# OzAmram/CaloDiffusion

Measured on AMD Instinct MI355X. Metric: sampled showers/sec (Dataset-2, 400-step DDIM), higher is better.
Workload: dtype f32 (convs: fp32 operands as 2-term fp16 splits on the fp16 MFMA pipe, fp32 accumulate; attention/norms fp32)

## Files before the change

### calodiffusion_amd/csrc/gn_defer.h

```cpp
#pragma once
#include "kernels_gn.h"

namespace cd {

__host__ __device__ inline int gn_defer_scratch_bytes(int C) { return C * 16 + 64 * 8; }

__device__ __forceinline__ void gn_defer_to_lds(const GnDefer& g, int b, float* coef_lds, void* scratch) {
  double* sC = (double*)scratch;
  float* sMR = (float*)((char*)scratch + g.C * 16);
  const int tid = threadIdx.x, nthreads = blockDim.x;
  const int C = g.C, G = g.groups;
  float pg = 0.f, pb = 0.f, pa = 0.f;
  if (tid < C) {
    pg = g.gamma[tid];
    pb = g.beta[tid];
    pa = g.add ? g.add[(size_t)b * g.add_ld + tid] : 0.f;
  }
  for (int i = tid; i < C * 8; i += nthreads) {
    const int c = i >> 3, j = i & 7;
    const float* p = g.part + ((size_t)b * g.units * C + c) * 2;
    double a1 = 0.0, a2 = 0.0;
    for (int u = j; u < g.units; u += 32) {
      float2 v[4];
#pragma unroll
      for (int k = 0; k < 4; ++k) v[k] = u + 8 * k < g.units ? *(const float2*)(p + (size_t)(u + 8 * k) * C * 2) : float2{0.f, 0.f};
#pragma unroll
      for (int k = 0; k < 4; ++k) {
        if (u + 8 * k < g.units) {
          a1 += (double)v[k].x;
          a2 += (double)v[k].y;
        }
      }
    }
#pragma unroll
    for (int m = 1; m < 8; m <<= 1) {
      a1 += __shfl_xor(a1, m, 64);
      a2 += __shfl_xor(a2, m, 64);
    }
    if (j == 0) {
      sC[c * 2] = a1;
      sC[c * 2 + 1] = a2;
    }
  }
  __syncthreads();
  const int cpg = C / G;
  if (tid < G) {
    double a1 = 0.0, a2 = 0.0;
    for (int c = 0; c < cpg; ++c) {
      a1 += sC[(tid * cpg + c) * 2];
      a2 += sC[(tid * cpg + c) * 2 + 1];
    }
    const double cnt = (double)g.vox * cpg;
    const double mu = a1 / cnt;
    double var = a2 / cnt - mu * mu;
    var = var < 0.0 ? 0.0 : var;
    sMR[tid * 2] = (float)mu;
    sMR[tid * 2 + 1] = (float)(1.0 / sqrt(var + 1e-5));
    if (g.stat_out) {
      g.stat_out[((size_t)b * G + tid) * 2] = sMR[tid * 2];
      g.stat_out[((size_t)b * G + tid) * 2 + 1] = sMR[tid * 2 + 1];
    }
  }
  __syncthreads();
  for (int c = tid; c < C; c += nthreads) {
    const int gi = c / cpg;
    const bool pre = c == tid;
    const float sc = sMR[gi * 2 + 1] * (pre ? pg : g.gamma[c]);
    f32x4 o;
    o[0] = sc;
    o[1] = (pre ? pb : g.beta[c]) - sMR[gi * 2] * sc;
    o[2] = pre ? pa : (g.add ? g.add[(size_t)b * g.add_ld + c] : 0.f);
    o[3] = 0.f;
    *(f32x4*)(coef_lds + c * 4) = o;
    if (g.coef_out) *(f32x4*)(g.coef_out + ((size_t)b * C + c) * 4) = o;
  }
  __syncthreads();
}

}
```

### calodiffusion_amd/csrc/kernels_conv_flat16.hip

```cpp
#include "conv_internal.h"
#include "gn_defer.h"

namespace cd {

template <int VT, int CT, int KD, int KH, int KW, int SZ, int SXY, int NTERM>
__global__ void __launch_bounds__(512, (VT * CT * (NTERM == 2 ? 2 : 1) <= 2 ? 3 : 2)) conv3_flat_bf16x3_kernel(ConvFlatArgs a) {
  extern __shared__ __attribute__((aligned(16))) float lds[];
  char* ldsb = (char*)lds;
  constexpr int T = KD * KH * KW;
  constexpr int VB = NTERM == 3 ? 96 : 80;
  constexpr int WS = 64 * NTERM;
  const int tid = threadIdx.x, lane = tid & 63, wave = tid >> 6, nthreads = blockDim.x;
  const int b = blockIdx.y;
  const int ct0 = blockIdx.z * CT;
  const int HW = a.H * a.W;
  const int vox = a.D * HW;
  const int HWo = a.Ho * a.Wo;
  const int voxo = a.Do * HWo;
  const int v0 = blockIdx.x * a.R;
  const int vend = min(v0 + a.R, voxo);
  const float inv_hwo = 1.f / (float)HWo, inv_wo = 1.f / (float)a.Wo;
  auto fdiv = [](int x, float inv) { return (int)(((float)x + 0.5f) * inv); };
  const int zA = fdiv(v0, inv_hwo) * SZ - 1;
  const int zB = fdiv(vend - 1, inv_hwo) * SZ + KD - 2;
  const int nstage = (zB - zA + 1) * HW;
  const int NZ = a.P * HW;
  const int half = lane >> 5, col = lane & 31;
  if (a.defer.part) gn_defer_to_lds(a.defer, b, (float*)(ldsb + a.coef_lds_off), ldsb + a.coef_lds_off + a.defer.C * 16);
  const bool normed = a.coef || a.defer.part;
  if (tid < VB / 4) ((float*)(ldsb + (size_t)NZ * VB))[tid] = 0.f;

  int nb[VT], rowoff[VT][KH], ooff[VT];
  unsigned wmask[VT];
  bool any_valid = false;
#pragma unroll
  for (int vt = 0; vt < VT; ++vt) {
    const int v = v0 + (wave * VT + vt) * 32 + col;
    const bool valid = v < vend;
    const int vv = valid ? v : v0;
    const int oz = fdiv(vv, inv_hwo);
    const int r = vv - oz * HWo;
    const int oh = fdiv(r, inv_wo), ow = r - oh * a.Wo;
    const int ih0 = oh * SXY, iw0 = ow * SXY;
    nb[vt] = (oz * SZ - 1 - zA) * HW + ih0 * a.W + iw0;
    unsigned m = 0;
#pragma unroll
    for (int kh = 0; kh < KH; ++kh) {
      int ih = ih0 + kh - 1;
      ih = ih < 0 ? ih + a.H : (ih >= a.H ? ih - a.H : ih);
      ih = ih >= a.H ? ih - a.H : ih;
      rowoff[vt][kh] = (ih - ih0) * a.W;
    }
#pragma unroll
    for (int kw = 0; kw < KW; ++kw) {
      const int iw = iw0 + kw - 1;
      if (valid && iw >= 0 && iw < a.W) m |= 1u << kw;
    }
    wmask[vt] = m;
    ooff[vt] = valid ? v * a.cout : -1;
    any_valid |= valid;
  }
  const bool wave_active = __any(any_valid);

  f32x16 acc[VT][CT], accB[NTERM == 2 ? VT : 1][NTERM == 2 ? CT : 1];
#pragma unroll
  for (int vt = 0; vt < VT; ++vt)
#pragma unroll
    for (int ct = 0; ct < CT; ++ct)
#pragma unroll
      for (int r = 0; r < 16; ++r) {
        acc[vt][ct][r] = 0.f;
        if (NTERM == 2) accB[vt][ct][r] = 0.f;
      }

  float amax = 0.f;
  float gscale = 1.f, ginv = 1.f;
  if (NTERM == 2 && a.in_absmax) pow2_scale_for(*a.in_absmax, &gscale, &ginv);
  const int nsub = (a.c0 + a.c1) >> 4;
  const int gbase = zA * HW;
  const int nslots = nstage * 4;

  auto tap_voxel = [&](int vt, int tap) -> int {
#ifdef CD_FLAT_ABL_TAPS
    return nb[vt] + tap;
#endif
    const int kz = tap / (KH * KW), kh = (tap / KW) % KH, kw = tap % KW;
    const int n = nb[vt] + kz * HW + rowoff[vt][kh] + kw - 1;
    return ((wmask[vt] >> kw) & 1u) ? n : NZ;
  };

  for (int sc = 0; sc < nsub; ++sc) {
    const float* src;
    int ldc, coff;
    if (sc * 16 < a.c0) {
      src = a.in0; ldc = a.c0; coff = sc * 16;
    } else {
      src = a.in1; ldc = a.c1; coff = sc * 16 - a.c0;
    }
    const int pq = tid & 3;
    src += (size_t)b * vox * ldc + coff + pq * 4;
    f32x4 cf[4];
    if (a.defer.part) {
#pragma unroll
      for (int e = 0; e < 4; ++e) cf[e] = *(const f32x4*)(ldsb + a.coef_lds_off + (sc * 16 + pq * 4 + e) * 16);
    } else if (a.coef) {
#pragma unroll
      for (int e = 0; e < 4; ++e) cf[e] = *(const f32x4*)(a.coef + ((size_t)b * (a.c0 + a.c1) + sc * 16 + pq * 4 + e) * 4);
    }
    __syncthreads();
    for (int s0 = tid; s0 < ((a.dbg & 1) ? 0 : nslots); s0 += 4 * nthreads) {
      f32x4 val[4];
#pragma unroll
      for (int k = 0; k < 4; ++k) {
        const int sidx = s0 + k * nthreads;
        const int g = gbase + (sidx >> 2);
        val[k] = f32x4{0.f, 0.f, 0.f, 0.f};
        if (sidx < nslots && g >= 0 && g < vox) {
          val[k] = *(const f32x4*)(src + (size_t)g * ldc);
          if (normed) {
#pragma unroll
            for (int e = 0; e < 4; ++e) {
              float t = cf[e][0] * val[k][e] + cf[e][1];
              if (a.act) t = cd_fast_silu(t);
              val[k][e] = t + cf[e][2];
            }
          }
        }
      }
#pragma unroll
      for (int k = 0; k < 4; ++k) {
        const int sidx = s0 + k * nthreads;
        if (sidx < nslots) {
          char* d = ldsb + (size_t)(sidx >> 2) * VB + pq * 8;
          if (NTERM == 3) {
            u32x2 t1, t2, t3;
            split3(val[k], t1, t2, t3);
            *(u32x2*)d = t1;
            *(u32x2*)(d + 32) = t2;
            *(u32x2*)(d + 64) = t3;
          } else {
            const f32x4 vs = val[k] * gscale;
            amax = fmaxf(amax, fmaxf(fmaxf(fabsf(vs[0]), fabsf(vs[1])), fmaxf(fabsf(vs[2]), fabsf(vs[3]))));
            u32x2 t1, t2;
            split2(vs, t1, t2);
            *(u32x2*)d = t1;
            *(u32x2*)(d + 32) = t2;
          }
        }
      }
    }
    __syncthreads();
    if (!wave_active || (a.dbg & 2)) continue;

#pragma unroll
    for (int vt = 0; vt < VT; ++vt) asm volatile("" : "+v"(nb[vt]));

    const u32x4* wq = (const u32x4*)a.wpk + ((size_t)sc * T * a.CTtot + ct0) * WS + lane;
#ifndef CD_FLAT_WD
#define CD_FLAT_WD 3
#endif
#ifndef CD_FLAT_AD
#define CD_FLAT_AD 2
#endif
    constexpr bool DEEP = NTERM == 2;
    constexpr int WD = DEEP ? CD_FLAT_WD : 1, AD = DEEP ? CD_FLAT_AD : 1;
    u32x4 bw[WD + 1][CT][NTERM], av[AD + 1][VT][NTERM];
    auto load_w = [&](int tap) {
#pragma unroll
      for (int ct = 0; ct < CT; ++ct)
#pragma unroll
        for (int t = 0; t < NTERM; ++t) bw[tap % (WD + 1)][ct][t] = wq[((size_t)tap * a.CTtot + ct) * WS + t * 64];
    };
    auto load_a = [&](int tap) {
#pragma unroll
      for (int vt = 0; vt < VT; ++vt) {
        const char* p = ldsb + (size_t)tap_voxel(vt, tap) * VB + half * 16;
#pragma unroll
        for (int t = 0; t < NTERM; ++t) av[tap % (AD + 1)][vt][t] = *(const u32x4*)(p + t * 32);
      }
    };
#pragma unroll
    for (int t0 = 0; t0 < WD; ++t0) load_w(t0);
#pragma unroll
    for (int t0 = 0; t0 < AD; ++t0) load_a(t0);
#pragma unroll
    for (int tap = 0; tap < T; ++tap) {
      if (tap + WD < T) load_w(tap + WD);
      if (tap + AD < T) load_a(tap + AD);
      __builtin_amdgcn_sched_barrier(0);
      const int wc = tap % (WD + 1), ac = tap % (AD + 1);
#pragma unroll
      for (int vt = 0; vt < VT; ++vt)
#pragma unroll
        for (int ct = 0; ct < CT; ++ct) {
          if (NTERM == 3) {
            f32x16 c = acc[vt][ct];
            c = MFMA_BF16(av[ac][vt][NTERM - 1], bw[wc][ct][0], c);
            c = MFMA_BF16(av[ac][vt][1], bw[wc][ct][1], c);
            c = MFMA_BF16(av[ac][vt][0], bw[wc][ct][NTERM - 1], c);
            c = MFMA_BF16(av[ac][vt][1], bw[wc][ct][0], c);
            c = MFMA_BF16(av[ac][vt][0], bw[wc][ct][1], c);
            c = MFMA_BF16(av[ac][vt][0], bw[wc][ct][0], c);
            acc[vt][ct] = c;
          } else {
            acc[vt][ct] = MFMA_F16(av[ac][vt][0], bw[wc][ct][0], acc[vt][ct]);
            accB[vt][ct] = MFMA_F16(av[ac][vt][0], bw[wc][ct][1], accB[vt][ct]);
            accB[vt][ct] = MFMA_F16(av[ac][vt][1], bw[wc][ct][0], accB[vt][ct]);
          }
        }
    }
  }

  if (NTERM == 2) {
#pragma unroll
    for (int vt = 0; vt < VT; ++vt)
#pragma unroll
      for (int ct = 0; ct < CT; ++ct)
#pragma unroll
        for (int r = 0; r < 16; ++r) acc[vt][ct][r] = (acc[vt][ct][r] + accB[vt][ct][r] * (1.f / 2048.f)) * ginv;
  }
  if (NTERM == 2 && a.status && amax > 65504.f) atomicOr(a.status, 1);
  float* outb = a.out + (size_t)b * voxo * a.cout;
  float bv[CT];
#pragma unroll
  for (int ct = 0; ct < CT; ++ct) bv[ct] = a.bias ? a.bias[(ct0 + ct) * 32 + col] : 0.f;
  if (a.add_src) {
    const float* addb = a.add_src + (size_t)b * voxo * a.cout;
#pragma unroll
    for (int vt = 0; vt < VT; ++vt) {
      float ad[16][CT];
#pragma unroll
      for (int r = 0; r < 16; ++r) {
        const int off = __shfl(ooff[vt], (r & 3) + 8 * (r >> 2) + 4 * half, 64);
#pragma unroll
        for (int ct = 0; ct < CT; ++ct) ad[r][ct] = off >= 0 ? addb[off + (ct0 + ct) * 32 + col] : 0.f;
      }
#pragma unroll
      for (int r = 0; r < 16; ++r)
#pragma unroll
        for (int ct = 0; ct < CT; ++ct) acc[vt][ct][r] += ad[r][ct];
    }
  }
#pragma unroll
  for (int vt = 0; vt < VT; ++vt) {
#pragma unroll
    for (int r = 0; r < 16; ++r) {
      const int row = (r & 3) + 8 * (r >> 2) + 4 * half;
      const int off = __shfl(ooff[vt], row, 64);
      if (off >= 0) {
#pragma unroll
        for (int ct = 0; ct < CT; ++ct) outb[off + (ct0 + ct) * 32 + col] = acc[vt][ct][r] + bv[ct];
      }
    }
  }
  if (a.ch_part) {
    float s1[CT], s2[CT];
#pragma unroll
    for (int ct = 0; ct < CT; ++ct) s1[ct] = s2[ct] = 0.f;
#pragma unroll
    for (int vt = 0; vt < VT; ++vt)
#pragma unroll
      for (int r = 0; r < 16; ++r) {
        const int row = (r & 3) + 8 * (r >> 2) + 4 * half;
        const bool ok = __shfl(ooff[vt], row, 64) >= 0;
#pragma unroll
        for (int ct = 0; ct < CT; ++ct) {
          const float v = ok ? acc[vt][ct][r] + bv[ct] : 0.f;
          s1[ct] += v;
          s2[ct] += v * v;
        }
      }
    __syncthreads();
    const int nw = nthreads >> 6;
#pragma unroll
    for (int ct = 0; ct < CT; ++ct) {
      const float t1 = s1[ct] + __shfl_xor(s1[ct], 32, 64), t2 = s2[ct] + __shfl_xor(s2[ct], 32, 64);
      if (half == 0) {
        lds[((wave * CT + ct) * 32 + col) * 2] = t1;
        lds[((wave * CT + ct) * 32 + col) * 2 + 1] = t2;
      }
    }
    __syncthreads();
    for (int i = tid; i < CT * 32; i += nthreads) {
      float t1 = 0.f, t2 = 0.f;
      for (int w = 0; w < nw; ++w) {
        t1 += lds[((w * CT * 32) + i) * 2];
        t2 += lds[((w * CT * 32) + i) * 2 + 1];
      }
      float* dst = a.ch_part + (((size_t)b * gridDim.x + blockIdx.x) * a.cout + ct0 * 32 + i) * 2;
      dst[0] = t1;
      dst[1] = t2;
    }
  }
}

namespace {
template <int VT, int CT, int KD, int KH, int KW, int SZ, int SXY, int NTERM>
void launch_flat3_geo(const ConvFlatArgs& a, dim3 grid, int threads, size_t lds, hipStream_t s) {
  static bool attr_set = false;
  if (!attr_set) {
    CD_HIP(hipFuncSetAttribute((const void*)conv3_flat_bf16x3_kernel<VT, CT, KD, KH, KW, SZ, SXY, NTERM>,
                               hipFuncAttributeMaxDynamicSharedMemorySize, 160 * 1024));
    attr_set = true;
  }
  hipLaunchKernelGGL((conv3_flat_bf16x3_kernel<VT, CT, KD, KH, KW, SZ, SXY, NTERM>), grid, dim3(threads), lds, s, a);
  CD_HIP(hipGetLastError());
}
template <int VT, int CT, int NTERM>
void launch_flat3_inst(const ConvFlatArgs& a, dim3 grid, int threads, size_t lds, hipStream_t s, int geo = 0) {
  if (geo == 0) launch_flat3_geo<VT, CT, 3, 3, 3, 1, 1, NTERM>(a, grid, threads, lds, s);
  else if (geo == 1) launch_flat3_geo<VT, CT, 3, 4, 4, 2, 2, NTERM>(a, grid, threads, lds, s);
  else if (geo == 2) launch_flat3_geo<VT, CT, 3, 4, 4, 1, 2, NTERM>(a, grid, threads, lds, s);
  else launch_flat3_geo<VT, CT, 4, 4, 4, 2, 2, NTERM>(a, grid, threads, lds, s);
}
}

bool launch_conv_flat_split16(int VT, int CT, int NTERM, int geo, const ConvFlatArgs& a, dim3 grid, int threads, size_t lds, hipStream_t s) {
#define CD_FLAT_CASE(V, C)                                                                 \
  if (VT == V && CT == C) {                                                                \
    if (NTERM == 3) launch_flat3_inst<V, C, 3>(a, grid, threads, lds, s, geo);             \
    else if constexpr (V * C <= 4) launch_flat3_inst<V, C, 2>(a, grid, threads, lds, s, geo); \
    else return false;                                                                     \
    return true;                                                                           \
  }
  CD_FLAT_CASE(1, 1) CD_FLAT_CASE(2, 1) CD_FLAT_CASE(3, 1) CD_FLAT_CASE(4, 1)
  CD_FLAT_CASE(1, 2) CD_FLAT_CASE(2, 2) CD_FLAT_CASE(3, 2) CD_FLAT_CASE(4, 2)
  CD_FLAT_CASE(1, 3) CD_FLAT_CASE(2, 3)
#undef CD_FLAT_CASE
  return false;
}

}
```

### calodiffusion_amd/csrc/kernels_gn.hip

```cpp
#include "kernels_gn.h"
#include "gn_defer.h"
#include <cstdio>
#include <cstdlib>

namespace cd {

int gn_nsplit_for(int64_t vox, int batch) {
  static const int target = getenv("CD_GN_NSPLIT_TARGET") ? atoi(getenv("CD_GN_NSPLIT_TARGET")) : 2048;
  int64_t want = (target + batch - 1) / batch;
  int64_t cap = (vox + 255) / 256;
  int64_t n = want < cap ? want : cap;
  if (n < 1) n = 1;
  if (n > 64) n = 64;
  return (int)n;
}

__global__ void __launch_bounds__(256) ch_stats_kernel(const float* __restrict__ x, float* __restrict__ part, int channels,
                                                       int64_t vox, int nsplit) {
  __shared__ double sP[256][2];
  const int tid = threadIdx.x;
  const int split = blockIdx.x, b = blockIdx.y;
  const int cols = channels >> 2;
  const int rows = 256 / cols;
  const int64_t per = (vox + nsplit - 1) / nsplit;
  const int64_t v0 = split * per;
  const int64_t v1 = (v0 + per < vox) ? v0 + per : vox;
  const int colid = tid % cols, row = tid / cols;
  f32x4 s1 = {0.f, 0.f, 0.f, 0.f}, s2 = {0.f, 0.f, 0.f, 0.f};
  if (row < rows) {
    const float* base = x + (size_t)b * vox * channels + colid * 4;
    for (int64_t v = v0 + row; v < v1; v += rows) {
      const f32x4 t = *(const f32x4*)(base + (size_t)v * channels);
      s1 += t;
      s2 += t * t;
    }
  }
  float* dst = part + (((size_t)b * nsplit + split) * channels) * 2;
  for (int e = 0; e < 4; ++e) {
    sP[tid][0] = (double)s1[e];
    sP[tid][1] = (double)s2[e];
    __syncthreads();
    if (tid < cols) {
      double a1 = 0.0, a2 = 0.0;
      for (int r = 0; r < rows; ++r) {
        a1 += sP[r * cols + tid][0];
        a2 += sP[r * cols + tid][1];
      }
      dst[(tid * 4 + e) * 2] = (float)a1;
      dst[(tid * 4 + e) * 2 + 1] = (float)a2;
    }
    __syncthreads();
  }
}

void launch_ch_stats(const float* x, float* part, int batch, int channels, int64_t vox, int nsplit, hipStream_t s) {
  CD_REQUIRE(channels % 4 == 0 && channels <= 256, "channel stats: channels must be a multiple of 4 and <= 256");
  char cat[64];
  std::snprintf(cat, sizeof cat, "ch_stats C%d n%ld", channels, (long)vox);
  prof::Scope scope(cat, s, 0, 4.0 * batch * (double)vox * channels);
  hipLaunchKernelGGL(ch_stats_kernel, dim3(nsplit, batch), dim3(256), 0, s, x, part, channels, vox, nsplit);
  CD_HIP(hipGetLastError());
}

__global__ void __launch_bounds__(256) gn_finalize_kernel(const float* __restrict__ part, int units, const float* __restrict__ gamma,
                                                          const float* __restrict__ beta, const float* __restrict__ add_bc,
                                                          int add_ld, float* __restrict__ coef, int channels, int groups,
                                                          int64_t vox, float* __restrict__ stat_out) {
  __shared__ double sS[256][2];
  __shared__ double sC[256][2];
  __shared__ float sMean[64], sRstd[64];
  const int b = blockIdx.x, tid = threadIdx.x;
  const int nsl = 256 / channels;
  const int c = tid % channels, sl = tid / channels;
  if (sl < nsl) {
    const float* p = part + ((size_t)b * units * channels + c) * 2;
    double a1 = 0.0, a2 = 0.0;
    for (int u = sl; u < units; u += nsl) {
      const float2 v = *(const float2*)(p + (size_t)u * channels * 2);
      a1 += (double)v.x;
      a2 += (double)v.y;
    }
    sS[tid][0] = a1;
    sS[tid][1] = a2;
  }
  __syncthreads();
  if (tid < channels) {
    double a1 = 0.0, a2 = 0.0;
    for (int k = 0; k < nsl; ++k) {
      a1 += sS[k * channels + tid][0];
      a2 += sS[k * channels + tid][1];
    }
    sC[tid][0] = a1;
    sC[tid][1] = a2;
  }
  __syncthreads();
  const int cpg = channels / groups;
  if (tid < groups) {
    double a1 = 0.0, a2 = 0.0;
    for (int c = 0; c < cpg; ++c) {
      a1 += sC[tid * cpg + c][0];
      a2 += sC[tid * cpg + c][1];
    }
    const double cnt = (double)vox * cpg;
    const double mu = a1 / cnt;
    double var = a2 / cnt - mu * mu;
    var = var < 0.0 ? 0.0 : var;
    sMean[tid] = (float)mu;
    sRstd[tid] = (float)(1.0 / sqrt(var + 1e-5));
    if (stat_out) {
      stat_out[((size_t)b * groups + tid) * 2] = sMean[tid];
      stat_out[((size_t)b * groups + tid) * 2 + 1] = sRstd[tid];
    }
  }
  __syncthreads();
  if (tid < channels) {
    const int g = tid / cpg;
    const float sc = sRstd[g] * gamma[tid];
    f32x4 o;
    o[0] = sc;
    o[1] = beta[tid] - sMean[g] * sc;
    o[2] = add_bc ? add_bc[(size_t)b * add_ld + tid] : 0.f;
    o[3] = 0.f;
    *(f32x4*)(coef + ((size_t)b * channels + tid) * 4) = o;
  }
}

void launch_gn_finalize(const float* part, int units, const float* gamma, const float* beta, const float* add_bc, int add_ld,
                        float* coef, int batch, int channels, int groups, int64_t vox, hipStream_t s, float* stat_out) {
  CD_REQUIRE(channels <= 256 && groups <= 64 && channels % groups == 0, "group norm: <= 256 channels, <= 64 groups");
  prof::Scope scope("gn_finalize", s, 0, 0);
  hipLaunchKernelGGL(gn_finalize_kernel, dim3(batch), dim3(256), 0, s, part, units, gamma, beta, add_bc, add_ld, coef, channels,
                     groups, vox, stat_out);
  CD_HIP(hipGetLastError());
}

__global__ void __launch_bounds__(256) gn_apply_kernel(const float* __restrict__ x, float* __restrict__ y,
                                                       const float* __restrict__ coef, int channels, int64_t vox, int silu,
                                                       const float* __restrict__ residual,
                                                       const float* __restrict__ residual1, int res_c0,
                                                       int blocks_per_sample, float* __restrict__ part_out, GnDefer defer) {
  __shared__ double sP[256][2];
  __shared__ __attribute__((aligned(16))) float sCoef[256 * 4];
  __shared__ __attribute__((aligned(16))) char sDefer[256 * 16 + 64 * 8];
  if (defer.part) gn_defer_to_lds(defer, blockIdx.x / blocks_per_sample, sCoef, sDefer);
  const int tid = threadIdx.x;
  const int b = blockIdx.x / blocks_per_sample, blk = blockIdx.x % blocks_per_sample;
  const int cols = channels >> 2;
  const int rows = 256 / cols;
  const int64_t vper = (vox + blocks_per_sample - 1) / blocks_per_sample;
  const int64_t v0 = blk * vper;
  const int64_t v1 = (v0 + vper < vox) ? v0 + vper : vox;
  const int colid = tid % cols, row = tid / cols;
  const int c = colid * 4;
  f32x4 s1 = {0.f, 0.f, 0.f, 0.f}, s2 = {0.f, 0.f, 0.f, 0.f};
  if (row < rows) {
    f32x4 cf[4];
#pragma unroll
    for (int e = 0; e < 4; ++e)
      cf[e] = defer.part ? *(const f32x4*)(sCoef + (c + e) * 4) : *(const f32x4*)(coef + ((size_t)b * channels + c + e) * 4);
    const size_t sbase = (size_t)b * vox * channels;
    const int res_c1 = channels - res_c0;
    auto act = [&](f32x4 t) {
#pragma unroll
      for (int e = 0; e < 4; ++e) {
        float u = cf[e][0] * t[e] + cf[e][1];
        if (silu) u = u * __builtin_amdgcn_rcpf(1.f + __builtin_amdgcn_exp2f(u * -1.4426950408889634f));
        t[e] = u + cf[e][2];
      }
      return t;
    };
    auto res_at = [&](int64_t v) {
      if (residual1)
        return c < res_c0 ? *(const f32x4*)(residual + ((size_t)b * vox + v) * res_c0 + c)
                          : *(const f32x4*)(residual1 + ((size_t)b * vox + v) * res_c1 + (c - res_c0));
      return *(const f32x4*)(residual + sbase + (size_t)v * channels + c);
    };
    int64_t v = v0 + row;
    for (; v + 3 * rows < v1; v += 4 * rows) {
      f32x4 t[4], r[4];
#pragma unroll
      for (int u = 0; u < 4; ++u) t[u] = *(const f32x4*)(x + sbase + (size_t)(v + u * rows) * channels + c);
      if (residual) {
#pragma unroll
        for (int u = 0; u < 4; ++u) r[u] = res_at(v + u * rows);
      }
#pragma unroll
      for (int u = 0; u < 4; ++u) {
        f32x4 o = act(t[u]);
        if (residual) o += r[u];
        *(f32x4*)(y + sbase + (size_t)(v + u * rows) * channels + c) = o;
        s1 += o;
        s2 += o * o;
      }
    }
    for (; v < v1; v += rows) {
      f32x4 o = act(*(const f32x4*)(x + sbase + (size_t)v * channels + c));
      if (residual) o += res_at(v);
      *(f32x4*)(y + sbase + (size_t)v * channels + c) = o;
      s1 += o;
      s2 += o * o;
    }
  }
  if (part_out) {
    float* dst = part_out + (((size_t)b * blocks_per_sample + blk) * channels) * 2;
    for (int e = 0; e < 4; ++e) {
      sP[tid][0] = (double)s1[e];
      sP[tid][1] = (double)s2[e];
      __syncthreads();
      if (tid < cols) {
        double a1 = 0.0, a2 = 0.0;
        for (int r = 0; r < rows; ++r) {
          a1 += sP[r * cols + tid][0];
          a2 += sP[r * cols + tid][1];
        }
        dst[(tid * 4 + e) * 2] = (float)a1;
        dst[(tid * 4 + e) * 2 + 1] = (float)a2;
      }
      __syncthreads();
    }
  }
}

int gn_apply_blocks_per_sample(int batch, int channels, int64_t vox) {
  const int rows = 256 / (channels / 4);
  int64_t bps = (vox + (int64_t)rows * 8 - 1) / ((int64_t)rows * 8);
  static const int target = getenv("CD_GN_APPLY_WGS") ? atoi(getenv("CD_GN_APPLY_WGS")) : 1024;
  const int64_t want = (target + batch - 1) / batch;
  if (bps > want) bps = want;
  if (bps < 1) bps = 1;
  return (int)bps;
}

void launch_gn_apply(const float* x, float* y, const float* coef, int batch, int channels, int64_t vox, int silu,
                     const float* residual, const float* residual1, int res_c0, float* part_out, hipStream_t s,
                     const GnDefer* defer) {
  CD_REQUIRE(channels % 4 == 0 && channels <= 256, "group norm: channels must be a multiple of 4 and <= 256");
  CD_REQUIRE(!defer || !defer->part || (defer->C == channels && defer->groups <= 64), "gn_apply: bad deferred normalisation");
  const int bps = gn_apply_blocks_per_sample(batch, channels, vox);
  char cat[64];
  std::snprintf(cat, sizeof cat, "gn_apply C%d n%ld", channels, (long)vox);
  prof::Scope scope(cat, s, 0, 4.0 * batch * (double)vox * channels * (2 + (residual ? 1 : 0)));
  hipLaunchKernelGGL(gn_apply_kernel, dim3((unsigned)(batch * bps)), dim3(256), 0, s, x, y, coef, channels, vox, silu, residual,
                     residual1, res_c0, bps, part_out, defer ? *defer : GnDefer());
  CD_HIP(hipGetLastError());
}

}
```

### calodiffusion_amd/csrc/kernels_pointwise.hip

```cpp
#include "conv_internal.h"
#include "gn_defer.h"

namespace cd {

template <int CT, int PRO>
__global__ void __launch_bounds__(256) pointwise_kernel(PointwiseArgs a, int CTtot) {
  const int tid = threadIdx.x, lane = tid & 63, wave = tid >> 6;
  const int half = lane >> 5, col = lane & 31;
  const int b = blockIdx.y;
  const int ct0 = blockIdx.z * CT;
  const int64_t n0 = (int64_t)blockIdx.x * 128 + wave * 32;
  const int64_t n = n0 + col;
  const bool valid = n < a.vox;

  __shared__ __attribute__((aligned(16))) float sGn[128 * 4];
  __shared__ __attribute__((aligned(16))) char sGnScratch[128 * 16 + 64 * 8];
  float hv[CT][16];
  const bool full = n0 + 32 <= a.vox && (ct0 + CT) * 32 <= a.cout;
  const int rl = 4 * half;
  if (a.gn_res) {
    gn_defer_to_lds(a.gn_defer, b, sGn, sGnScratch);
    if (full) {
      const float* hp = a.gn_res + ((size_t)b * a.vox + n0) * a.cout + ct0 * 32 + col;
#pragma unroll
      for (int ct = 0; ct < CT; ++ct)
#pragma unroll
        for (int r = 0; r < 16; ++r) hv[ct][r] = hp[((r & 3) + 8 * (r >> 2) + rl) * a.cout + ct * 32];
    } else {
#pragma unroll
      for (int ct = 0; ct < CT; ++ct) {
        const int co = min((ct0 + ct) * 32 + col, a.cout - 1);
#pragma unroll
        for (int r = 0; r < 16; ++r) {
          const int64_t nr = min(n0 + (r & 3) + 8 * (r >> 2) + 4 * half, a.vox - 1);
          hv[ct][r] = a.gn_res[((size_t)b * a.vox + nr) * a.cout + co];
        }
      }
    }
  }

  f32x16 acc[CT];
#pragma unroll
  for (int ct = 0; ct < CT; ++ct)
#pragma unroll
    for (int r = 0; r < 16; ++r) acc[ct][r] = 0.f;

  const int nchunk = (a.c0 + a.c1) >> 5;
  const float* wb = a.wpk + (size_t)b * a.w_batch_stride;
  if (PRO == A_NONE && a.wpk16) {
    f32x16 accB[CT];
#pragma unroll
    for (int ct = 0; ct < CT; ++ct)
#pragma unroll
      for (int r = 0; r < 16; ++r) accB[ct][r] = 0.f;
    float amax = 0.f;
    for (int chunk = 0; chunk < nchunk; ++chunk) {
      const float* src;
      if (chunk * 32 < a.c0) src = a.in0 + ((size_t)b * a.vox + (valid ? n : 0)) * a.ld0 + a.off0 + chunk * 32 + half * 16;
      else src = a.in1 + ((size_t)b * a.vox + (valid ? n : 0)) * a.ld1 + (chunk * 32 - a.c0) + half * 16;
      f32x4 av[4];
#pragma unroll
      for (int q = 0; q < 4; ++q) {
        av[q] = *(const f32x4*)(src + q * 4);
        if (!valid) av[q] = f32x4{0.f, 0.f, 0.f, 0.f};
        amax = fmaxf(fmaxf(fmaxf(amax, fabsf(av[q][0])), fabsf(av[q][1])), fmaxf(fabsf(av[q][2]), fabsf(av[q][3])));
      }
#pragma unroll
      for (int ks = 0; ks < 2; ++ks) {
        u32x2 h0, l0, h1, l1;
        split2(av[2 * ks], h0, l0);
        split2(av[2 * ks + 1], h1, l1);
        const u32x4 a1 = {h0[0], h0[1], h1[0], h1[1]}, a2 = {l0[0], l0[1], l1[0], l1[1]};
        const u32x4* wp = (const u32x4*)a.wpk16 + ((size_t)(chunk * 2 + half) * CTtot + ct0) * 128 + ks * 32 + col;
#pragma unroll
        for (int ct = 0; ct < CT; ++ct) {
          const u32x4 w1 = wp[ct * 128], w2 = wp[ct * 128 + 64];
          acc[ct] = MFMA_F16(a1, w1, acc[ct]);
          accB[ct] = MFMA_F16(a1, w2, accB[ct]);
          accB[ct] = MFMA_F16(a2, w1, accB[ct]);
        }
      }
    }
#pragma unroll
    for (int ct = 0; ct < CT; ++ct)
#pragma unroll
      for (int r = 0; r < 16; ++r) acc[ct][r] += accB[ct][r] * (1.f / 2048.f);
    if (a.status && amax > 65504.f) atomicOr(a.status, 1);
  } else
  for (int chunk = 0; chunk < nchunk; ++chunk) {
    const float* src;
    if (chunk * 32 < a.c0) src = a.in0 + ((size_t)b * a.vox + (valid ? n : 0)) * a.ld0 + a.off0 + chunk * 32 + half * 16;
    else src = a.in1 + ((size_t)b * a.vox + (valid ? n : 0)) * a.ld1 + (chunk * 32 - a.c0) + half * 16;
    f32x4 av[4];
#pragma unroll
    for (int q = 0; q < 4; ++q) {
      av[q] = *(const f32x4*)(src + q * 4);
      if (!valid) av[q] = f32x4{0.f, 0.f, 0.f, 0.f};
    }
    if (PRO == A_AFFINE) {
      const float* cfp = a.coef + ((size_t)b * (a.c0 + a.c1) + chunk * 32 + half * 16) * 4;
#pragma unroll
      for (int q = 0; q < 4; ++q)
#pragma unroll
        for (int e = 0; e < 4; ++e) {
          const f32x4 cf = *(const f32x4*)(cfp + (q * 4 + e) * 4);
          av[q][e] = cf[0] * av[q][e] + cf[1];
        }
    } else if (PRO == A_EXPNORM) {
      const float* cfp = a.coef + ((size_t)b * (a.c0 + a.c1) + chunk * 32 + half * 16) * 2;
#pragma unroll
      for (int q = 0; q < 4; ++q)
#pragma unroll
        for (int e = 0; e < 4; ++e) av[q][e] = valid ? expf(av[q][e] - cfp[(q * 4 + e) * 2]) * cfp[(q * 4 + e) * 2 + 1] : 0.f;
    } else if (PRO == A_SOFTMAX32) {
      float m = av[0][0];
#pragma unroll
      for (int q = 0; q < 4; ++q)
#pragma unroll
        for (int e = 0; e < 4; ++e) m = fmaxf(m, av[q][e]);
      m = fmaxf(m, __shfl_xor(m, 32, 64));
      float ssum = 0.f;
#pragma unroll
      for (int q = 0; q < 4; ++q)
#pragma unroll
        for (int e = 0; e < 4; ++e) {
          av[q][e] = expf(av[q][e] - m);
          ssum += av[q][e];
        }
      ssum += __shfl_xor(ssum, 32, 64);
      const float inv = 1.f / ssum;
#pragma unroll
      for (int q = 0; q < 4; ++q)
#pragma unroll
        for (int e = 0; e < 4; ++e) av[q][e] *= inv;
    }
    const f32x4* wq = (const f32x4*)wb + ((size_t)chunk * CTtot + ct0) * 256 + lane;
#pragma unroll
    for (int ct = 0; ct < CT; ++ct) {
      f32x4 bw[4];
#pragma unroll
      for (int q = 0; q < 4; ++q) bw[q] = wq[ct * 256 + q * 64];
#pragma unroll
      for (int q = 0; q < 4; ++q)
#pragma unroll
        for (int e = 0; e < 4; ++e) acc[ct] = MFMA32(av[q][e], bw[q][e], acc[ct]);
    }
  }

  if (full) {
    const int ld = a.out_ld ? a.out_ld : a.cout;
    __shared__ __attribute__((aligned(16))) float sTr[4][32 * 36];
    float* tr = sTr[wave];
    float* op = a.out + ((size_t)b * a.vox + n0) * ld + a.out_off + ct0 * 32 + (lane & 7) * 4;
    const float* rp = a.residual ? a.residual + ((size_t)b * a.vox + n0) * a.cout + ct0 * 32 + col : nullptr;
#pragma unroll
    for (int ct = 0; ct < CT; ++ct) {
      const float bv = a.bias ? a.bias[(ct0 + ct) * 32 + col] : 0.f;
      f32x4 cf = {0.f, 0.f, 0.f, 0.f};
      if (a.gn_res) cf = *(const f32x4*)(sGn + ((ct0 + ct) * 32 + col) * 4);
      float rv[16];
      if (rp) {
#pragma unroll
        for (int r = 0; r < 16; ++r) rv[r] = rp[((r & 3) + 8 * (r >> 2) + rl) * a.cout + ct * 32];
      }
#pragma unroll
      for (int r = 0; r < 16; ++r) {
        float v = acc[ct][r] + bv;
        if (rp) v += rv[r];
        if (a.gn_res) {
          const float u = cf[0] * hv[ct][r] + cf[1];
          v += u * __builtin_amdgcn_rcpf(1.f + __builtin_amdgcn_exp2f(u * -1.4426950408889634f)) + cf[2];
        }
        acc[ct][r] = v;
        tr[((r & 3) + 8 * (r >> 2) + rl) * 36 + col] = v;
      }
      asm volatile("s_waitcnt lgkmcnt(0)" ::: "memory");
#pragma unroll
      for (int k = 0; k < 4; ++k) {
        const int row = 8 * k + (lane >> 3);
        *(f32x4*)(op + (size_t)row * ld + ct * 32) = *(const f32x4*)(tr + row * 36 + (lane & 7) * 4);
      }
      if (ct + 1 < CT) asm volatile("s_waitcnt lgkmcnt(0)" ::: "memory");
    }
  } else {
#pragma unroll
  for (int ct = 0; ct < CT; ++ct) {
    const int co = (ct0 + ct) * 32 + col;
    const bool cok = co < a.cout;
    const float bv = (a.bias && cok) ? a.bias[co] : 0.f;
    f32x4 cf = {0.f, 0.f, 0.f, 0.f};
    if (a.gn_res && cok) cf = *(const f32x4*)(sGn + co * 4);
#pragma unroll
    for (int r = 0; r < 16; ++r) {
      const int64_t nr = n0 + (r & 3) + 8 * (r >> 2) + 4 * half;
      float v = acc[ct][r] + bv;
      if (a.residual && cok && nr < a.vox) v += a.residual[((size_t)b * a.vox + nr) * a.cout + co];
      if (a.gn_res) {
        const float u = cf[0] * hv[ct][r] + cf[1];
        v += u * __builtin_amdgcn_rcpf(1.f + __builtin_amdgcn_exp2f(u * -1.4426950408889634f)) + cf[2];
      }
      acc[ct][r] = v;
    }
  }
#pragma unroll
  for (int r = 0; r < 16; ++r) {
    const int row = (r & 3) + 8 * (r >> 2) + 4 * half;
    const int64_t nr = n0 + row;
    if (nr < a.vox) {
#pragma unroll
      for (int ct = 0; ct < CT; ++ct) {
        const int co = (ct0 + ct) * 32 + col;
        if (co < a.cout) a.out[((size_t)b * a.vox + nr) * (a.out_ld ? a.out_ld : a.cout) + a.out_off + co] = acc[ct][r];
      }
    }
  }
  }
  if (a.ch_part) {
    __shared__ float red[4][CT * 32][2];
#pragma unroll
    for (int ct = 0; ct < CT; ++ct) {
      float s1 = 0.f, s2 = 0.f;
#pragma unroll
      for (int r = 0; r < 16; ++r) {
        const int row = (r & 3) + 8 * (r >> 2) + 4 * half;
        if (full || n0 + row < a.vox) {
          const float v = acc[ct][r];
          s1 += v;
          s2 += v * v;
        }
      }
      s1 += __shfl_xor(s1, 32, 64);
      s2 += __shfl_xor(s2, 32, 64);
      if (half == 0) {
        red[wave][ct * 32 + col][0] = s1;
        red[wave][ct * 32 + col][1] = s2;
      }
    }
    __syncthreads();
    if (tid < CT * 32 && ct0 * 32 + tid < a.cout) {
      const float t1 = (red[0][tid][0] + red[1][tid][0]) + (red[2][tid][0] + red[3][tid][0]);
      const float t2 = (red[0][tid][1] + red[1][tid][1]) + (red[2][tid][1] + red[3][tid][1]);
      float* dst = a.ch_part + (((size_t)b * gridDim.x + blockIdx.x) * a.cout + ct0 * 32 + tid) * 2;
      dst[0] = t1;
      dst[1] = t2;
    }
  }
}

void launch_pointwise(const PointwiseArgs& a, hipStream_t s) {
  CD_REQUIRE(a.c0 % 32 == 0 && a.c1 % 32 == 0 && a.c0 > 0, "pointwise conv: channels must be multiples of 32");
  CD_REQUIRE(a.prologue != A_SOFTMAX32 || (a.c0 == 32 && a.c1 == 0), "softmax prologue needs exactly 32 channels");
  CD_REQUIRE(!a.gn_res || (a.gn_defer.part && a.gn_defer.C == a.cout && a.cout <= 128 && !a.out_ld),
             "pointwise conv: the fused block close normalises a packed tensor of the output's width (<= 128 channels)");
  CD_REQUIRE(a.out_off % 4 == 0 && a.out_ld % 4 == 0 && (a.cout % 4 == 0 || a.out_ld), "pointwise conv: output rows must be 16-byte aligned");
  CD_REQUIRE(!a.wpk16 || (a.prologue == A_NONE && !a.w_batch_stride && a.cout % 32 == 0),
             "pointwise conv: the fp16-pipe form takes shared weights, whole 32-channel tiles and no input prologue");
  const int CTtot = (a.cout + 31) / 32;
  const int CT = CTtot <= 3 ? CTtot : (CTtot % 2 == 0 ? 2 : 1);
  dim3 grid((unsigned)((a.vox + 127) / 128), (unsigned)a.batch, (unsigned)(CTtot / CT));
  char cat[128];
  std::snprintf(cat, sizeof cat, "pointwise_p%d C%d->%d n%ld", a.prologue, a.c0 + a.c1, a.cout, (long)a.vox);
  prof::Scope scope(cat, s, 2.0 * (a.c0 + a.c1) * a.cout * (double)a.vox * a.batch,
                    4.0 * a.batch * (double)a.vox * (a.c0 + a.c1 + a.cout + (a.residual ? a.cout : 0)));
#define CD_PW_CASE(C, P)                                                                   \
  if (CT == C && a.prologue == P) {                                                        \
    hipLaunchKernelGGL((pointwise_kernel<C, P>), grid, dim3(256), 0, s, a, CTtot);         \
    CD_HIP(hipGetLastError());                                                             \
    return;                                                                                \
  }
  CD_PW_CASE(1, A_NONE) CD_PW_CASE(2, A_NONE) CD_PW_CASE(3, A_NONE)
  CD_PW_CASE(1, A_AFFINE) CD_PW_CASE(2, A_AFFINE) CD_PW_CASE(3, A_AFFINE)
  CD_PW_CASE(1, A_SOFTMAX32) CD_PW_CASE(2, A_SOFTMAX32) CD_PW_CASE(3, A_SOFTMAX32)
  CD_PW_CASE(1, A_EXPNORM) CD_PW_CASE(2, A_EXPNORM) CD_PW_CASE(3, A_EXPNORM)
#undef CD_PW_CASE
  CD_REQUIRE(false, "pointwise conv: no kernel instance");
}

}
```

Baseline: 94.41.

## Fold GroupNorm finalize per channel and overlap it with loads

Rewrites the deferred GroupNorm coefficient computation so each channel thread computes its own group mean and rstd. This drops one barrier and the tid<G serial stage, and the partial-sum loop now issues 8 loads per trip instead of 4. In the GN apply, pointwise and small conv kernels, the first global loads are issued before the fold and the trailing barrier is delayed, so load latency overlaps the stats reduction. Groups are now reduced redundantly once per channel, which adds LDS reads and register pressure.

Measured after the change: 94.43 (median of 3 runs). Within noise of the previous version (+0.0%).

```diff
diff --git a/calodiffusion_amd/csrc/gn_defer.h b/calodiffusion_amd/csrc/gn_defer.h
--- a/calodiffusion_amd/csrc/gn_defer.h
+++ b/calodiffusion_amd/csrc/gn_defer.h
@@ -4,6 +4,81 @@
 namespace cd {
 
 __host__ __device__ inline int gn_defer_scratch_bytes(int C) { return C * 16 + 64 * 8; }
+
+#ifndef CD_GN_FOLD_V1
+
+__device__ __forceinline__ void gn_defer_fold(const GnDefer& g, int b, float* coef_lds, void* scratch) {
+  double* sC = (double*)scratch;
+  const int tid = threadIdx.x, nthreads = blockDim.x;
+  const int C = g.C, G = g.groups, units = g.units;
+  float pg = 0.f, pb = 0.f, pa = 0.f;
+  if (tid < C) {
+    pg = g.gamma[tid];
+    pb = g.beta[tid];
+    pa = g.add ? g.add[(size_t)b * g.add_ld + tid] : 0.f;
+  }
+  for (int i = tid; i < C * 8; i += nthreads) {
+    const int c = i >> 3, j = i & 7;
+    const float* p = g.part + ((size_t)b * units * C + c) * 2;
+    double a1 = 0.0, a2 = 0.0;
+    for (int u = j; u < units; u += 64) {
+      float2 v[8];
+#pragma unroll
+      for (int k = 0; k < 8; ++k) v[k] = u + 8 * k < units ? *(const float2*)(p + (size_t)(u + 8 * k) * C * 2) : float2{0.f, 0.f};
+#pragma unroll
+      for (int k = 0; k < 8; ++k) {
+        if (u + 8 * k < units) {
+          a1 += (double)v[k].x;
+          a2 += (double)v[k].y;
+        }
+      }
+    }
+#pragma unroll
+    for (int m = 1; m < 8; m <<= 1) {
+      a1 += __shfl_xor(a1, m, 64);
+      a2 += __shfl_xor(a2, m, 64);
+    }
+    if (j == 0) {
+      sC[c * 2] = a1;
+      sC[c * 2 + 1] = a2;
+    }
+  }
+  __syncthreads();
+  const int cpg = C / G;
+  for (int c = tid; c < C; c += nthreads) {
+    const int gi = c / cpg;
+    double a1 = 0.0, a2 = 0.0;
+    for (int cc = 0; cc < cpg; ++cc) {
+      a1 += sC[(gi * cpg + cc) * 2];
+      a2 += sC[(gi * cpg + cc) * 2 + 1];
+    }
+    const double cnt = (double)g.vox * cpg;
+    const double mu = a1 / cnt;
+    double var = a2 / cnt - mu * mu;
+    var = var < 0.0 ? 0.0 : var;
+    const float mean = (float)mu, rstd = (float)(1.0 / sqrt(var + 1e-5));
+    if (g.stat_out && c == gi * cpg) {
+      g.stat_out[((size_t)b * G + gi) * 2] = mean;
+      g.stat_out[((size_t)b * G + gi) * 2 + 1] = rstd;
+    }
+    const bool pre = c == tid;
+    const float sc = rstd * (pre ? pg : g.gamma[c]);
+    f32x4 o;
+    o[0] = sc;
+    o[1] = (pre ? pb : g.beta[c]) - mean * sc;
+    o[2] = pre ? pa : (g.add ? g.add[(size_t)b * g.add_ld + c] : 0.f);
+    o[3] = 0.f;
+    *(f32x4*)(coef_lds + c * 4) = o;
+    if (g.coef_out) *(f32x4*)(g.coef_out + ((size_t)b * C + c) * 4) = o;
+  }
+}
+
+__device__ __forceinline__ void gn_defer_to_lds(const GnDefer& g, int b, float* coef_lds, void* scratch) {
+  gn_defer_fold(g, b, coef_lds, scratch);
+  __syncthreads();
+}
+
+#else
 
 __device__ __forceinline__ void gn_defer_to_lds(const GnDefer& g, int b, float* coef_lds, void* scratch) {
   double* sC = (double*)scratch;
@@ -77,4 +152,6 @@
   __syncthreads();
 }
 
+#endif
+
 }
diff --git a/calodiffusion_amd/csrc/kernels_conv_flat16.hip b/calodiffusion_amd/csrc/kernels_conv_flat16.hip
--- a/calodiffusion_amd/csrc/kernels_conv_flat16.hip
+++ b/calodiffusion_amd/csrc/kernels_conv_flat16.hip
@@ -26,7 +26,16 @@
   const int nstage = (zB - zA + 1) * HW;
   const int NZ = a.P * HW;
   const int half = lane >> 5, col = lane & 31;
+#ifdef CD_GN_FOLD_V1
+  constexpr bool LATE_CF = false;
   if (a.defer.part) gn_defer_to_lds(a.defer, b, (float*)(ldsb + a.coef_lds_off), ldsb + a.coef_lds_off + a.defer.C * 16);
+#else
+  constexpr bool LATE_CF = NTERM == 2 && VT * CT == 1;
+  if (a.defer.part) {
+    if (LATE_CF) gn_defer_fold(a.defer, b, (float*)(ldsb + a.coef_lds_off), ldsb + a.coef_lds_off + a.defer.C * 16);
+    else gn_defer_to_lds(a.defer, b, (float*)(ldsb + a.coef_lds_off), ldsb + a.coef_lds_off + a.defer.C * 16);
+  }
+#endif
   const bool normed = a.coef || a.defer.part;
   if (tid < VB / 4) ((float*)(ldsb + (size_t)NZ * VB))[tid] = 0.f;
 
@@ -101,13 +110,19 @@
     src += (size_t)b * vox * ldc + coff + pq * 4;
     f32x4 cf[4];
     if (a.defer.part) {
+      if (!LATE_CF) {
+#pragma unroll
+        for (int e = 0; e < 4; ++e) cf[e] = *(const f32x4*)(ldsb + a.coef_lds_off + (sc * 16 + pq * 4 + e) * 16);
+      }
+    } else if (a.coef) {
+#pragma unroll
+      for (int e = 0; e < 4; ++e) cf[e] = *(const f32x4*)(a.coef + ((size_t)b * (a.c0 + a.c1) + sc * 16 + pq * 4 + e) * 4);
+    }
+    __syncthreads();
+    if (LATE_CF && a.defer.part) {
 #pragma unroll
       for (int e = 0; e < 4; ++e) cf[e] = *(const f32x4*)(ldsb + a.coef_lds_off + (sc * 16 + pq * 4 + e) * 16);
-    } else if (a.coef) {
-#pragma unroll
-      for (int e = 0; e < 4; ++e) cf[e] = *(const f32x4*)(a.coef + ((size_t)b * (a.c0 + a.c1) + sc * 16 + pq * 4 + e) * 4);
-    }
-    __syncthreads();
+    }
     for (int s0 = tid; s0 < ((a.dbg & 1) ? 0 : nslots); s0 += 4 * nthreads) {
       f32x4 val[4];
 #pragma unroll
diff --git a/calodiffusion_amd/csrc/kernels_gn.hip b/calodiffusion_amd/csrc/kernels_gn.hip
--- a/calodiffusion_amd/csrc/kernels_gn.hip
+++ b/calodiffusion_amd/csrc/kernels_gn.hip
@@ -142,7 +142,9 @@
   __shared__ double sP[256][2];
   __shared__ __attribute__((aligned(16))) float sCoef[256 * 4];
   __shared__ __attribute__((aligned(16))) char sDefer[256 * 16 + 64 * 8];
+#ifdef CD_GN_FOLD_V1
   if (defer.part) gn_defer_to_lds(defer, blockIdx.x / blocks_per_sample, sCoef, sDefer);
+#endif
   const int tid = threadIdx.x;
   const int b = blockIdx.x / blocks_per_sample, blk = blockIdx.x % blocks_per_sample;
   const int cols = channels >> 2;
@@ -153,6 +155,15 @@
   const int colid = tid % cols, row = tid / cols;
   const int c = colid * 4;
   f32x4 s1 = {0.f, 0.f, 0.f, 0.f}, s2 = {0.f, 0.f, 0.f, 0.f};
+#ifndef CD_GN_FOLD_V1
+  f32x4 t0[4];
+  const bool first_trip = row < rows && v0 + row + 3 * rows < v1;
+  if (first_trip) {
+#pragma unroll
+    for (int u = 0; u < 4; ++u) t0[u] = *(const f32x4*)(x + ((size_t)b * vox + v0 + row + u * rows) * channels + c);
+  }
+  if (defer.part) gn_defer_to_lds(defer, b, sCoef, sDefer);
+#endif
   if (row < rows) {
     f32x4 cf[4];
 #pragma unroll
@@ -178,8 +189,16 @@
     int64_t v = v0 + row;
     for (; v + 3 * rows < v1; v += 4 * rows) {
       f32x4 t[4], r[4];
-#pragma unroll
-      for (int u = 0; u < 4; ++u) t[u] = *(const f32x4*)(x + sbase + (size_t)(v + u * rows) * channels + c);
+#ifndef CD_GN_FOLD_V1
+      if (v == v0 + row) {
+#pragma unroll
+        for (int u = 0; u < 4; ++u) t[u] = t0[u];
+      } else
+#endif
+      {
+#pragma unroll
+        for (int u = 0; u < 4; ++u) t[u] = *(const f32x4*)(x + sbase + (size_t)(v + u * rows) * channels + c);
+      }
       if (residual) {
 #pragma unroll
         for (int u = 0; u < 4; ++u) r[u] = res_at(v + u * rows);
diff --git a/calodiffusion_amd/csrc/kernels_pointwise.hip b/calodiffusion_amd/csrc/kernels_pointwise.hip
--- a/calodiffusion_amd/csrc/kernels_pointwise.hip
+++ b/calodiffusion_amd/csrc/kernels_pointwise.hip
@@ -19,7 +19,9 @@
   const bool full = n0 + 32 <= a.vox && (ct0 + CT) * 32 <= a.cout;
   const int rl = 4 * half;
   if (a.gn_res) {
+#ifdef CD_GN_FOLD_V1
     gn_defer_to_lds(a.gn_defer, b, sGn, sGnScratch);
+#endif
     if (full) {
       const float* hp = a.gn_res + ((size_t)b * a.vox + n0) * a.cout + ct0 * 32 + col;
 #pragma unroll
@@ -37,6 +39,9 @@
         }
       }
     }
+#ifndef CD_GN_FOLD_V1
+    gn_defer_fold(a.gn_defer, b, sGn, sGnScratch);
+#endif
   }
 
   f32x16 acc[CT];
@@ -147,6 +152,9 @@
     }
   }
 
+#ifndef CD_GN_FOLD_V1
+  if (a.gn_res) __syncthreads();
+#endif
   if (full) {
     const int ld = a.out_ld ? a.out_ld : a.cout;
     __shared__ __attribute__((aligned(16))) float sTr[4][32 * 36];
```
